# netapp-rickhuang-ai/spark-rapids-ml-nai

Hardware: AMD Instinct MI355X
Metric: fit-time speedup vs Spark-ML CPU (geomean over reference headline workloads, 1Mx3000 fp32) (higher is better)
Workload: dtype fp32

## Files before the change

spark_rapids_ml_nai_amd/ops/__init__.py:

```python
from __future__ import annotations

import math
import os
from typing import Any, Dict, Iterator, Optional, Tuple

import numpy as np
import torch

from . import native
from ..utils.determinism import deterministic

__all__ = ["col_moments", "gram", "xw", "dgemm", "sign_flip", "is_native", "xtv", "row_sqnorm",
           "logreg_binary_loss_grad", "nearest_centroid", "cluster_sums", "csr_logreg_binary_loss_grad",
           "csr_spmm", "csr_spmtm", "csr_col_moments", "logistic_loss_grad"]


def is_native(t: torch.Tensor) -> bool:
    return t.is_cuda


def _c(t: torch.Tensor) -> torch.Tensor:
    return t if t.is_contiguous() else t.contiguous()


# ... 419 lines not shown
    return labels, dist


_CERTIFY_STATS = {"rows": 0, "refined": 0}


F16_U = 2.0 ** -11
F16_A = 2.0 ** -14


def certify_tau16(n: int) -> float:
    return 1.01 * (2.0 * F16_U + F16_U * F16_U + 1.01 * float(n) * 2.0 ** -24)


def f16_radius_terms(n: int, scale: float, tau: float) -> Tuple[float, float, float]:
    a = F16_A / scale
    z = 2.02 * a * math.sqrt(n) * (1.0 + F16_U)
    z2 = 2.02 * float(n) * a * a
    wmax = math.sqrt(n) * 32768.0 / scale
    return (z + 2.0 ** -24 * wmax) / (2.0 * tau), z, z2


class F16Planes:

    def __init__(self, X: torch.Tensor, mu: torch.Tensor) -> None:
        m, n = X.shape
        self.X, self.m, self.n = X, m, n
        self.mu = _c(mu.float().view(-1))
        dev = X.device
        st = native.stream(dev)
        self.xnorm = torch.empty(m, dtype=torch.float32, device=dev)
        amax = zeros(1, dtype=torch.int32, device=dev)
        native.call("srml_row_sqnorm_centered_amax_f32", X.data_ptr(), m, n, X.stride(0), self.mu.data_ptr(),
                    self.xnorm.data_ptr(), amax.data_ptr(), st)
        a = float(amax.view(torch.float32).item())
        self.ok = math.isfinite(a) and a > 0.0
        self.scale = 1.0
        self.P = None
        if not self.ok:
            return
        e = math.frexp(a)[1] - 1
        if not -100 <= 13 - e <= 100:
            self.ok = False
            return
        self.scale = 2.0 ** (13 - e)
        self.kp = (n + 15) // 16 * 16
        self.rows_pad = max(256, (m + 255) // 256 * 256)
        self.P = torch.empty((self.rows_pad // 256, self.kp // 16, 256, 16), dtype=torch.float16, device=dev)
        self.ovf = zeros(1, dtype=torch.int32, device=dev)
        native.call("srml_split_f16_tiled_centered", X.data_ptr(), m, n, X.stride(0), self.mu.data_ptr(), self.kp,
                    self.rows_pad, self.scale, self.P.data_ptr(), self.ovf.data_ptr(), st)
        self.tau = certify_tau16(n)
        self.xadd, self.z, self.z2 = f16_radius_terms(n, self.scale, self.tau)


F16_CAND_CAP = 64


def _f16_centre_planes(F: F16Planes, C: torch.Tensor, approx: bool) -> Tuple[torch.Tensor, ...]:
    k, dev = C.shape[0], F.X.device
    st = native.stream(dev)
    Cd = _c(C.to(dev)) if C.dtype in (torch.float32, torch.float64) else _c(C.to(dev, torch.float32))
    crows = max(256, (k + 255) // 256 * 256)
    W = torch.empty((k, F.n), dtype=torch.float32, device=dev)
    cn = torch.empty(crows, dtype=torch.float32, device=dev)
    cg = torch.empty(k, dtype=torch.float32, device=dev)
    zero2 = torch.empty(2, dtype=torch.int32, device=dev)
    native.call("srml_f16_centre_prep", Cd.data_ptr(), int(Cd.dtype == torch.float64), k, F.n, F.mu.data_ptr(),
                float(2.0 * F.tau), int(bool(approx)), W.data_ptr(), cn.data_ptr(), cg.data_ptr(), zero2.data_ptr(), st)
    CP = torch.empty((crows // 256, F.kp // 16, 256, 16), dtype=torch.float16, device=dev)
    native.call("srml_split_f16_tiled_centered", W.data_ptr(), k, F.n, W.stride(0), None, F.kp, crows, F.scale,
                CP.data_ptr(), zero2[0:1].data_ptr(), st)
    return W, cn, cg, zero2, CP, crows


def nearest_f16_labels(F: F16Planes, C: torch.Tensor) -> Optional[torch.Tensor]:
    if F.kp != 128 or os.environ.get("SRML_F16_ROWLOOP", "1") == "0":
        return None
    dev = F.X.device
    _, cn, _, _, CP, crows = _f16_centre_planes(F, C, True)
    labels = torch.empty(F.m, dtype=torch.int32, device=dev)
    rc = native.lib().srml_nearest_f16_rowloop(F.P.data_ptr(), F.m, F.rows_pad, F.kp, CP.data_ptr(), C.shape[0],
                                                crows, cn.data_ptr(), float(-2.0 / (F.scale * F.scale)),
                                                labels.data_ptr(), native.stream(dev))
    if rc == -2:
        return None
    if rc != 0:
        raise RuntimeError("srml_nearest_f16_rowloop failed (%d)" % rc)
    return labels


def nearest_centroid_f16(F: F16Planes, C: torch.Tensor, approx: bool = False) -> Tuple[torch.Tensor, torch.Tensor]:
    m, k, dev = F.m, C.shape[0], F.X.device
    st = native.stream(dev)
    W, cn, cg, zero2, CP, crows = _f16_centre_planes(F, C, approx)
    ovf = zero2[0:1]
    xadd, z, z2 = (0.0, 0.0, 0.0) if approx else (F.xadd, F.z, F.z2)
    dscale = -2.0 / (F.scale * F.scale)
    nslot = int(native.lib().srml_nearest_centroid_f16_top2_nslot(k))
    labels = torch.empty(m, dtype=torch.int32, device=dev)
    dist = torch.empty(m, dtype=torch.float32, device=dev)
    flagged = torch.empty(m, dtype=torch.int32, device=dev)
    thr = torch.empty(m, dtype=torch.float32, device=dev)
    cnt = zero2[1:2]
    step = split_rows_per_launch(k)
    for r0 in range(0, m, step):
# ... 2147 lines not shown
```

spark_rapids_ml_nai_amd/ops/csrc/splitmm.hip:

```cpp
#include "common.h"

#include "tile.h"
#include <stdlib.h>

namespace {
using srml_tile::orderable;
using srml_tile::unorderable;

typedef short bf16x8 __attribute__((ext_vector_type(8)));
typedef _Float16 halfx8 __attribute__((ext_vector_type(8)));
typedef unsigned uintx4 __attribute__((ext_vector_type(4)));
typedef unsigned uintx2 __attribute__((ext_vector_type(2)));

__device__ __forceinline__ unsigned bf16_rn(float f) {
  unsigned u = __float_as_uint(f);
  u += 0x7fffu + ((u >> 16) & 1u);
  return u >> 16;
}
__device__ __forceinline__ float bf16_f(unsigned b) { return __uint_as_float(b << 16); }

__global__ __launch_bounds__(256) void split_kernel(const float* __restrict__ X, long m, int n, long ld, int kp,
                                                    long rows_pad, unsigned short* __restrict__ P) {
  const int q4 = kp >> 2;
  const long total = rows_pad * q4;
  const long plane = rows_pad * (long)kp;
  for (long i = (long)blockIdx.x * 256 + threadIdx.x; i < total; i += (long)gridDim.x * 256) {
    const long r = i / q4;
    const int c = (int)(i - r * q4) * 4;
    unsigned h[4], md[4], lo[4];
#pragma unroll
    for (int j = 0; j < 4; ++j) {
      const float x = (r < m && c + j < n) ? X[r * ld + c + j] : 0.f;
      h[j] = bf16_rn(x);
      const float r1 = x - bf16_f(h[j]);
      md[j] = bf16_rn(r1);
      lo[j] = bf16_rn(r1 - bf16_f(md[j]));
    }
    const long o = r * kp + c;
    *reinterpret_cast<uintx2*>(P + o) = uintx2{h[0] | (h[1] << 16), h[2] | (h[3] << 16)};
    *reinterpret_cast<uintx2*>(P + plane + o) = uintx2{md[0] | (md[1] << 16), md[2] | (md[3] << 16)};
    *reinterpret_cast<uintx2*>(P + 2 * plane + o) = uintx2{lo[0] | (lo[1] << 16), lo[2] | (lo[3] << 16)};
  }
}

__global__ __launch_bounds__(256) void split_tiled_kernel(const float* __restrict__ X, long m, int n, long ld, int kp,
                                                          long rows_pad, unsigned short* __restrict__ P,
                                                          const float* __restrict__ mu,
                                                          const int* __restrict__ ridx = nullptr) {
  const int ks_n = kp >> 4;
  const long total = rows_pad * ks_n;
  const long plane = rows_pad * (long)kp;
  const bool vec = (ld & 3) == 0 && (reinterpret_cast<uintptr_t>(X) & 15) == 0;
  for (long i = (long)blockIdx.x * 256 + threadIdx.x; i < total; i += (long)gridDim.x * 256) {
    const long img = i >> 8;
    const int rr = (int)(i & 255);
    const long tile = img / ks_n;
    const int c0 = (int)(img - tile * ks_n) * 16;
    const long r = tile * 256 + rr;
    const long rs = ridx && r < m ? (long)ridx[r] : r;
    float x[16];
    if (vec && r < m && c0 + 16 <= n) {
#pragma unroll
      for (int q = 0; q < 4; ++q) {
        const floatx4 v = *reinterpret_cast<const floatx4*>(X + rs * ld + c0 + 4 * q);
        x[4 * q] = v[0]; x[4 * q + 1] = v[1]; x[4 * q + 2] = v[2]; x[4 * q + 3] = v[3];
// ... 368 lines not shown
    for (int p = 0; p < 3; ++p) {
      a[p] = *reinterpret_cast<const uintx4*>(xa + p * xplane + ko);
      b[p] = *reinterpret_cast<const uintx4*>(ca + p * cplane + ko);
    }
  };
  auto lstore = [&](int stage, const uintx4 (&a)[3], const uintx4 (&b)[3]) {
#pragma unroll
    for (int p = 0; p < 3; ++p) {
      *reinterpret_cast<uintx4*>(&st[stage].A[p][sr][sh]) = a[p];
      *reinterpret_cast<uintx4*>(&st[stage].B[p][sr][sh]) = b[p];
    }
  };
  const int nk = kp / SBK;
  if (PF == 1) {
    uintx4 ra[3], rb[3];
    gload(0, ra, rb);
    lstore(0, ra, rb);
    __syncthreads();
    int cur = 0;
    for (int kt = 0; kt < nk; ++kt) {
      const bool more = kt + 1 < nk;
      if (more) gload(kt + 1, ra, rb);
      mma_step(cur);
      if (more) lstore(cur ^ 1, ra, rb);
      __syncthreads();
      cur ^= 1;
    }
  } else {
    uintx4 ra0[3], rb0[3], ra1[3], rb1[3];
    gload(0, ra0, rb0);
    if (nk > 1) gload(1, ra1, rb1);
    lstore(0, ra0, rb0);
    __syncthreads();
    int kt = 0;
    for (; kt + 2 <= nk; kt += 2) {
      if (kt + 2 < nk) gload(kt + 2, ra0, rb0);
      mma_step(0);
      lstore(1, ra1, rb1);
      __syncthreads();
      if (kt + 3 < nk) gload(kt + 3, ra1, rb1);
      mma_step(1);
      if (kt + 2 < nk) lstore(0, ra0, rb0);
      __syncthreads();
    }
    if (kt < nk) mma_step(0);
  }

  split_epilogue<BM, BN, WM, WN>(acc, row0, col0, m, k, cnorm, best, wm, wn, li, lk);
}

typedef __attribute__((address_space(3))) void* lds_vptr;
typedef __attribute__((address_space(1))) void* gbl_vptr;

template <bool TILED, int NP = 6, bool TOP2 = false, int WN_ = 4, bool PRIO = false, bool CAND = false, int RING = 0>
__global__ __launch_bounds__(WN_ * 128, WN_ == 4 ? 1 : 2) void nearest_centroid_split_glds_kernel(
    const unsigned short* __restrict__ XP, long m, long xrows, int kp, const unsigned short* __restrict__ CP, int k,
    long crows, const float* __restrict__ cnorm, unsigned long long* __restrict__ best, int n_ctiles,
    float* __restrict__ lob = nullptr, const float* __restrict__ cg = nullptr, const float* __restrict__ xnorm = nullptr,
    float dscale = -2.f, float xadd = 0.f, const float* __restrict__ thr = nullptr, int* __restrict__ ccount = nullptr,
    int* __restrict__ cand = nullptr, int cap = 0) {
  static_assert(!CAND || (NP == 1 && TOP2), "candidate lists come from the fp16 filter");
  static_assert(WN_ == 4 || (WN_ == 2 && NP != 6), "256 x 128 tiles are built for the filter passes");
  static_assert(NP == 6 || NP == 3 || (NP == 1 && TOP2), "NP = 1 is the fp16 certified filter");
  constexpr int BM = 256, WM = 2, WN = WN_, BN = 64 * WN, TM = 4, TN = 2;
  constexpr int NPL = NP == 6 ? 3 : (NP == 3 ? 2 : 1);
  constexpr int XCH = NPL * (BM / 32), CCH = NPL * (BN / 32);
  constexpr int CPW = (XCH + CCH) / (WM * WN);
  static_assert((XCH + CCH) % (WM * WN) == 0, "chunks split evenly over the waves");
  constexpr int KPB = RING ? RING / 10 : NP == 1 ? 3 : (NP == 3 && WN_ == 4 ? 2 : 1);
  constexpr int NG = RING ? RING % 10 : NP == 1 && WN_ == 4 ? 3 : 2;
  static_assert(!RING || (NP == 1 && KPB >= 1 && NG >= 2), "ring override is for the fp16 filter");
  constexpr int NS = (KPB > 1 || RING) ? NG * KPB : 3;
  constexpr int STAGE = NPL * (BM + BN) * 16;
  __shared__ __attribute__((aligned(1024))) unsigned short lds[NS][STAGE];
  const int bid = xcd_remap(blockIdx.x, gridDim.x);
  const long rtile = bid / n_ctiles;
  const int ctile = bid % n_ctiles;
  const long row0 = rtile * BM;
  const int col0 = ctile * BN;
  const int t = threadIdx.x;
  const int lane = t & 63, wid = t >> 6;
  const int wm = wid / WN, wn = wid % WN;
  const int li = lane & 31, lk = lane >> 5;
  const long xplane = xrows * (long)kp, cplane = crows * (long)kp;

  const unsigned short* src[CPW];
  int dst_off[CPW];
#pragma unroll
  for (int i = 0; i < CPW; ++i) {
    const int c = wid * CPW + i;
    const bool isx = c < XCH;
    const int q = isx ? c / (BM / 32) : (c - XCH) / (BN / 32);
    const int j = isx ? c % (BM / 32) : (c - XCH) % (BN / 32);
    const int r = 32 * j + (lane >> 1);
    const int lh = (lane & 1) ^ ((lane >> 4) & 1);
    if (TILED) {
      const int ks_n = kp / SBK;
      if (isx) src[i] = XP + q * xplane + ((rtile * ks_n) << 12) + 512 * j + lane * 8;
      else src[i] = CP + q * cplane + (((long)(col0 >> 8) * ks_n) << 12) + 16 * (col0 & 255) + 512 * j + lane * 8;
    } else if (isx) {
      long xr = row0 + r;
      if (xr >= xrows) xr = xrows - 1;
      src[i] = XP + q * xplane + xr * kp + 8 * lh;
    } else {
      src[i] = CP + q * cplane + (long)(col0 + r) * kp + 8 * lh;
    }
    dst_off[i] = isx ? (q * BM + 32 * j) * 16 : (NPL * BM + q * BN + 32 * j) * 16;
  }
  auto issue = [&](int kt, int stage) {
    unsigned short* base = &lds[stage][0];
#pragma unroll
    for (int i = 0; i < CPW; ++i) {
      __builtin_amdgcn_global_load_lds((gbl_vptr)(src[i] + (TILED ? ((long)kt << 12) : (long)kt * SBK)),
                                       (lds_vptr)(base + dst_off[i]), 16, 0, 0);
    }
  };

  floatx16 acc[TM][TN];
#pragma unroll
  for (int a = 0; a < TM; ++a)
#pragma unroll
    for (int b = 0; b < TN; ++b)
#pragma unroll
      for (int r = 0; r < 16; ++r) acc[a][b][r] = 0.f;

  const int ph = lk ^ ((li >> 3) & 1);
  const int nk = kp / SBK;
  auto compute = [&](int st) {
    bf16x8 fb[NPL][TN];
#pragma unroll
    for (int p = 0; p < NPL; ++p)
#pragma unroll
      for (int nt = 0; nt < TN; ++nt)
        fb[p][nt] = *reinterpret_cast<const bf16x8*>(
            &lds[st][(NPL * BM + p * BN + wn * (BN / WN) + nt * 32 + li) * 16 + 8 * ph]);
#pragma unroll
    for (int mt = 0; mt < TM; ++mt) {
      bf16x8 fa[NPL];
#pragma unroll
      for (int p = 0; p < NPL; ++p)
        fa[p] = *reinterpret_cast<const bf16x8*>(&lds[st][(p * BM + wm * (BM / WM) + mt * 32 + li) * 16 + 8 * ph]);
#pragma unroll
      for (int nt = 0; nt < TN; ++nt) {
        if constexpr (NP == 1) {
          acc[mt][nt] = __builtin_amdgcn_mfma_f32_32x32x16_f16(__builtin_bit_cast(halfx8, fb[0][nt]),
                                                               __builtin_bit_cast(halfx8, fa[0]), acc[mt][nt], 0,
                                                               0, 0);
        } else {
          if constexpr (NP == 6) {
            acc[mt][nt] = __builtin_amdgcn_mfma_f32_32x32x16_bf16(fa[2], fb[0][nt], acc[mt][nt], 0, 0, 0);
            acc[mt][nt] = __builtin_amdgcn_mfma_f32_32x32x16_bf16(fa[1], fb[1][nt], acc[mt][nt], 0, 0, 0);
            acc[mt][nt] = __builtin_amdgcn_mfma_f32_32x32x16_bf16(fa[0], fb[2][nt], acc[mt][nt], 0, 0, 0);
          }
          acc[mt][nt] = __builtin_amdgcn_mfma_f32_32x32x16_bf16(fa[1], fb[0][nt], acc[mt][nt], 0, 0, 0);
          acc[mt][nt] = __builtin_amdgcn_mfma_f32_32x32x16_bf16(fa[0], fb[1][nt], acc[mt][nt], 0, 0, 0);
          acc[mt][nt] = __builtin_amdgcn_mfma_f32_32x32x16_bf16(fa[0], fb[0][nt], acc[mt][nt], 0, 0, 0);
        }
      }
    }
  };
  if constexpr (KPB == 1 && !RING) {
    static_assert(CPW == 6, "the counted wait below leaves one step (CPW loads) in flight");
    issue(0, 0);
    if (nk > 1) issue(1, 1);
    int stage = 0;
    for (int kt = 0; kt < nk; ++kt) {
      if (kt + 1 < nk) asm volatile("s_waitcnt vmcnt(6)" ::: "memory");
      else asm volatile("s_waitcnt vmcnt(0)" ::: "memory");
      __builtin_amdgcn_s_barrier();
      if (kt + 2 < nk) issue(kt + 2, stage == 0 ? 2 : stage - 1);
      if (PRIO) __builtin_amdgcn_s_setprio(1);
      compute(stage);
      if (PRIO) __builtin_amdgcn_s_setprio(0);
      stage = stage == 2 ? 0 : stage + 1;
    }
  } else {
#pragma unroll
    for (int j = 0; j < (NG - 1) * KPB; ++j)
      if (j < nk) issue(j, j);
    for (int kt = 0; kt < nk; kt += KPB) {
      if (NG >= 3 && kt + (NG - 1) * KPB <= nk)
        asm volatile("s_waitcnt vmcnt(%0)" ::"i"((NG - 2) * KPB * CPW) : "memory");
      else asm volatile("s_waitcnt vmcnt(0)" ::: "memory");
      __builtin_amdgcn_s_barrier();
#pragma unroll
      for (int j = 0; j < KPB; ++j)
        if (kt + (NG - 1) * KPB + j < nk) issue(kt + (NG - 1) * KPB + j, (kt + (NG - 1) * KPB + j) % NS);
      if (PRIO) __builtin_amdgcn_s_setprio(1);
#pragma unroll
      for (int j = 0; j < KPB; ++j)
        if (kt + j < nk) compute((kt + j) % NS);
      if (PRIO) __builtin_amdgcn_s_setprio(0);
    }
  }
  if (CAND)
    split_epilogue_cand_t<BM, BN, WM, WN>(acc, row0, col0, m, k, cnorm, cg, xnorm, wm, wn, li, lk, dscale, xadd, thr,
                                          ccount, cand, cap);
  else if (TOP2 && NP == 1)
    split_epilogue_top2_t<BM, BN, WM, WN>(acc, row0, col0, ctile, m, k, cnorm, cg, xnorm, best, lob, n_ctiles * WN, wm,
                                          wn, li, lk, dscale, xadd);
  else if (TOP2)
    split_epilogue_top2<BM, BN, WM, WN>(acc, row0, col0, ctile, m, k, cnorm, cg, xnorm, best, lob, n_ctiles * WN, wm,
                                        wn, li, lk, dscale, xadd);
  else
    split_epilogue<BM, BN, WM, WN>(acc, row0, col0, m, k, cnorm, best, wm, wn, li, lk);
}

__global__ __launch_bounds__(256) void split_top2_select_kernel(const unsigned long long* __restrict__ keys,
                                                                const float* __restrict__ lob, long m, int nslot,
                                                                const float* __restrict__ xnorm,
                                                                const float* __restrict__ cg,
                                                                int* __restrict__ labels, float* __restrict__ dist,
                                                                int* __restrict__ flagged, int* __restrict__ n_flagged,
                                                                float xadd = 0.f, float z = 0.f, float z2 = 0.f,
                                                                const int* __restrict__ ovf = nullptr,
                                                                float* __restrict__ thr_out = nullptr) {
  const long i = (long)blockIdx.x * 256 + threadIdx.x;
  if (i >= m) return;
  unsigned long long k1 = ~0ull;
  int s1 = 0;
  for (int s = 0; s < nslot; ++s) {
    const unsigned long long v = keys[(long)s * m + i];
    if (v < k1) { k1 = v; s1 = s; }
  }
  const float xn = xnorm[i];
  const float xs0 = sqrtf(fmaxf(xn, 0.f));
  const float xs = xs0 + xadd;
  const float c2 = 2.f * fmaf(z, xs0, z2);
  float low = __builtin_huge_valf();
  for (int s = 0; s < nslot; ++s) {
    low = fminf(low, lob[(long)s * m + i]);
    const unsigned long long v = keys[(long)s * m + i];
    if (s != s1 && v != ~0ull) low = fminf(low, fmaf(-xs, cg[(int)(v & 0xffffffffu)], unorderable((unsigned)(v >> 32))));
  }
  const float bv = unorderable((unsigned)(k1 >> 32));
  if (k1 != ~0ull && !(ovf && *ovf) && low > fmaf(xs, cg[(int)(k1 & 0xffffffffu)], bv) + c2) {
    labels[i] = (int)(k1 & 0xffffffffu);
    const float d = bv + xn;
    dist[i] = d > 0.f ? d : 0.f;
  } else {
    const int p = atomicAdd(n_flagged, 1);
    flagged[p] = (int)i;
    if (thr_out)
      thr_out[p] = (k1 != ~0ull && !(ovf && *ovf)) ? fmaf(xs, cg[(int)(k1 & 0xffffffffu)], bv) + c2
                                                   : __builtin_huge_valf();
  }
}
// ... 220 lines not shown
  return srml_nearest_centroid_split_tiled_np(XP, m, xrows, kp, CP, k, crows, cnorm, best, 6, stream);
}

SRML_API int srml_nearest_centroid_split_top2(const unsigned short* XP, long m, long xrows, int kp,
                                              const unsigned short* CP, int k, long crows, const float* cnorm,
                                              const float* cg, const float* xnorm, unsigned long long* keys,
                                              float* lob, hipStream_t stream) {
  if (m <= 0 || k <= 0) return 0;
  if ((kp & 15) || xrows < m || crows < k || (crows & 255) || (xrows & 255)) return -2;
  if ((reinterpret_cast<uintptr_t>(XP) & 15) || (reinterpret_cast<uintptr_t>(CP) & 15)) return -5;
  const long rt = (m + 255) / 256;
  const int bn = split3_bn();
  const int ct = (k + bn - 1) / bn;
  const long nb = rt * ct;
  if (nb > srml_max_blocks(512)) return -3;
  static const bool prio = !(getenv("SRML_SPLIT_PRIO") && atoi(getenv("SRML_SPLIT_PRIO")) == 0);
#define SRML_TOP2(WNN, PR, T)                                                                                    \
  hipLaunchKernelGGL((nearest_centroid_split_glds_kernel<true, 3, true, WNN, PR>), dim3((unsigned)nb), dim3(T), 0, \
                     stream, XP, m, xrows, kp, CP, k, crows, cnorm, keys, (int)ct, lob, cg, xnorm)
  if (bn == 128 && prio) SRML_TOP2(2, true, 256);
  else if (bn == 128) SRML_TOP2(2, false, 256);
  else if (prio) SRML_TOP2(4, true, 512);
  else SRML_TOP2(4, false, 512);
#undef SRML_TOP2
  return srml_status();
}

SRML_API int srml_nearest_centroid_split_top2_nslot(int k) {
  const int bn = split3_bn();
  return ((k + bn - 1) / bn) * (bn / 64);
}

SRML_API int srml_split_top2_select(const unsigned long long* keys, const float* lob, long m, int nslot,
                                    const float* xnorm, const float* cg, int* labels, float* dist, int* flagged,
                                    int* n_flagged, hipStream_t stream) {
  if (m <= 0) return 0;
  hipLaunchKernelGGL(split_top2_select_kernel, dim3((unsigned)((m + 255) / 256)), dim3(256), 0, stream, keys, lob, m,
                     nslot, xnorm, cg, labels, dist, flagged, n_flagged);
  return srml_status();
}

SRML_API int srml_split_scatter_refined(const unsigned long long* best, const int* rows, int nf, const float* xnorm,
                                        int* labels, float* dist, hipStream_t stream) {
  if (nf <= 0) return 0;
  hipLaunchKernelGGL(split_scatter_refined_kernel, dim3((unsigned)((nf + 255) / 256)), dim3(256), 0, stream, best,
                     rows, nf, xnorm, labels, dist);
  return srml_status();
}

static int f16_bn() {
  static const int bn = getenv("SRML_F16_BN") && atoi(getenv("SRML_F16_BN")) == 128 ? 128 : 256;
  return bn;
}
static int f16_slots_per_tile() { return f16_bn() / 64; }

template <typename T>
__global__ __launch_bounds__(256) void f16_centre_prep_kernel(const T* __restrict__ C, int k, int n,
                                                              const float* __restrict__ mu, float tau2, int approx,
                                                              float* __restrict__ W, float* __restrict__ cn,
                                                              float* __restrict__ cg, int* __restrict__ zero2) {
  const int j = blockIdx.x * 4 + (threadIdx.x >> 6);
  const int lane = threadIdx.x & 63;
  if (blockIdx.x == 0 && threadIdx.x < 2) zero2[threadIdx.x] = 0;
  if (j >= k) return;
  double a = 0.0;
  for (int d = lane; d < n; d += 64) {
    const float w = (float)((double)C[(long)j * n + d] - (double)mu[d]);
    W[(long)j * n + d] = w;
    a += (double)w * (double)w;
  }
  for (int o = 32; o > 0; o >>= 1) a += __shfl_xor(a, o, 64);
  if (lane == 0) {
    const float c = (float)a;
    cn[j] = c;
    cg[j] = approx ? 0.f : tau2 * sqrtf(c > 0.f ? c : 0.f);
  }
}

SRML_API int srml_f16_centre_prep(const void* C, int c_f64, int k, int n, const float* mu, float tau2, int approx,
                                  float* W, float* cn, float* cg, int* zero2, hipStream_t stream) {
  if (k <= 0) return 0;
  const dim3 grid((unsigned)((k + 3) / 4));
  if (c_f64)
    hipLaunchKernelGGL(f16_centre_prep_kernel<double>, grid, dim3(256), 0, stream,
                       reinterpret_cast<const double*>(C), k, n, mu, tau2, approx, W, cn, cg, zero2);
  else
    hipLaunchKernelGGL(f16_centre_prep_kernel<float>, grid, dim3(256), 0, stream, reinterpret_cast<const float*>(C),
                       k, n, mu, tau2, approx, W, cn, cg, zero2);
  return srml_status();
}

SRML_API int srml_split_f16_tiled_centered(const float* X, long m, int n, long ld, const float* mu, int kp,
                                           long rows_pad, float scale, unsigned short* P, int* ovf,
                                           hipStream_t stream) {
  if (rows_pad <= 0) return 0;
  if ((kp & 15) || kp < n || rows_pad < m || (rows_pad & 255)) return -2;
  if ((reinterpret_cast<uintptr_t>(P) & 15) != 0) return -5;
  const long total = rows_pad * (long)(kp / 16);
  long blocks = (total + 255) / 256;
  if (blocks > 65536) blocks = 65536;
  hipLaunchKernelGGL(split_tiled_f16_kernel, dim3((unsigned)blocks), dim3(256), 0, stream, X, m, n, ld, kp, rows_pad, P,
                     mu, scale, ovf);
  return srml_status();
}

SRML_API int srml_nearest_centroid_f16_top2(const unsigned short* XP, long m, long xrows, int kp,
                                            const unsigned short* CP, int k, long crows, const float* cnorm,
                                            const float* cg, const float* xnorm, float dscale, float xadd,
                                            unsigned long long* keys, float* lob, hipStream_t stream) {
  if (m <= 0 || k <= 0) return 0;
  if ((kp & 15) || xrows < m || crows < k || (crows & 255) || (xrows & 255)) return -2;
  if ((reinterpret_cast<uintptr_t>(XP) & 15) || (reinterpret_cast<uintptr_t>(CP) & 15)) return -5;
  const long rt = (m + 255) / 256;
  const int bn = f16_bn();
  const int ct = (k + bn - 1) / bn;
  const long nb = rt * ct;
  if (nb > srml_max_blocks(bn * 2)) return -3;
  static const bool prio = !(getenv("SRML_SPLIT_PRIO") && atoi(getenv("SRML_SPLIT_PRIO")) == 0);
#define SRML_F16(WNN, PR, T)                                                                                      \
  hipLaunchKernelGGL((nearest_centroid_split_glds_kernel<true, 1, true, WNN, PR>), dim3((unsigned)nb), dim3(T), 0, \
                     stream, XP, m, xrows, kp, CP, k, crows, cnorm, keys, (int)ct, lob, cg, xnorm, dscale, xadd)
  static const int ring = getenv("SRML_F16_RING") ? atoi(getenv("SRML_F16_RING")) : 0;
#define SRML_F16R(RG)                                                                                               \
  hipLaunchKernelGGL((nearest_centroid_split_glds_kernel<true, 1, true, 4, true, false, RG>), dim3((unsigned)nb),      \
                     dim3(512), 0, stream, XP, m, xrows, kp, CP, k, crows, cnorm, keys, (int)ct, lob, cg, xnorm,       \
                     dscale, xadd)
  if (f16_bn() == 128) {
    if (prio) SRML_F16(2, true, 256);
    else SRML_F16(2, false, 256);
  } else if (ring == 23) {
    SRML_F16R(23);
  } else if (ring == 24) {
    SRML_F16R(24);
  } else if (ring == 42) {
    SRML_F16R(42);
  } else if (ring == 18) {
    SRML_F16R(18);
  } else if (ring == 25) {
    SRML_F16R(25);
  } else {
    if (prio) SRML_F16(4, true, 512);
    else SRML_F16(4, false, 512);
  }
#undef SRML_F16R
#undef SRML_F16
  return srml_status();
}

SRML_API int srml_nearest_centroid_f16_top2_nslot(int k) {
  const int bn = f16_bn();
  return ((k + bn - 1) / bn) * f16_slots_per_tile();
}

SRML_API int srml_split_top2_select_f16(const unsigned long long* keys, const float* lob, long m, int nslot,
                                        const float* xnorm, const float* cg, float xadd, float z, float z2,
                                        const int* ovf, int* labels, float* dist, int* flagged, int* n_flagged,
                                        hipStream_t stream) {
  if (m <= 0) return 0;
  hipLaunchKernelGGL(split_top2_select_kernel, dim3((unsigned)((m + 255) / 256)), dim3(256), 0, stream, keys, lob, m,
                     nslot, xnorm, cg, labels, dist, flagged, n_flagged, xadd, z, z2, ovf);
  return srml_status();
}

SRML_API int srml_split_f16_tiled_centered_rows(const float* X, long ld, const int* ridx, long m, int n,
                                                const float* mu, int kp, long rows_pad, float scale, unsigned short* P,
                                                int* ovf, hipStream_t stream) {
  if (rows_pad <= 0) return 0;
  if ((kp & 15) || kp < n || rows_pad < m || (rows_pad & 255) || !ridx) return -2;
  if ((reinterpret_cast<uintptr_t>(P) & 15) != 0) return -5;
  const long total = rows_pad * (long)(kp / 16);
  long blocks = (total + 255) / 256;
  if (blocks > 65536) blocks = 65536;
  hipLaunchKernelGGL(split_tiled_f16_kernel, dim3((unsigned)blocks), dim3(256), 0, stream, X, m, n, ld, kp, rows_pad, P,
                     mu, scale, ovf, ridx);
  return srml_status();
}

__global__ __launch_bounds__(256) void f16_plane_gather_kernel(const uintx4* __restrict__ src, int ks_n,
                                                               const int* __restrict__ ridx, long m, long rows_pad,
                                                               uintx4* __restrict__ dst,
                                                               const float* __restrict__ xn = nullptr,
                                                               float* __restrict__ xn_out = nullptr,
                                                               int* __restrict__ zero_out = nullptr) {
  for (long i = (long)blockIdx.x * 256 + threadIdx.x; i < m; i += (long)gridDim.x * 256) {
    if (xn_out) xn_out[i] = xn[ridx[i]];
    if (zero_out) zero_out[i] = 0;
  }
  const long total = rows_pad * ks_n;
  for (long i = (long)blockIdx.x * 256 + threadIdx.x; i < total; i += (long)gridDim.x * 256) {
    const long img = i >> 8;
    const int rr = (int)(i & 255);
    const long tile = img / ks_n;
    const long ks = img - tile * ks_n;
    const long r = tile * 256 + rr;
    uintx4 lo = uintx4{0u, 0u, 0u, 0u}, hi = lo;
    if (r < m) {
// ... 2 lines not shown
      const uintx4* s = src + ((((rs >> 8) * ks_n + ks) << 12) + (rs & 255) * 16) / 8;
      lo = s[ssw];
      hi = s[ssw ^ 1];
    }
    const int dsw = (rr >> 3) & 1;
    uintx4* d = dst + ((img << 12) + rr * 16) / 8;
    d[dsw] = lo;
    d[dsw ^ 1] = hi;
  }
}

SRML_API int srml_f16_plane_gather_rows_ex(const unsigned short* P, long src_rows_pad, int kp, const int* ridx, long m,
                                           long rows_pad, unsigned short* out, const float* xn, float* xn_out,
                                           int* zero_out, hipStream_t stream) {
  if (rows_pad <= 0) return 0;
  if ((kp & 15) || rows_pad < m || (rows_pad & 255) || (src_rows_pad & 255) || !ridx) return -2;
  if ((reinterpret_cast<uintptr_t>(P) & 15) || (reinterpret_cast<uintptr_t>(out) & 15)) return -5;
  if (xn_out && !xn) return -2;
  const long total = rows_pad * (long)(kp / 16);
  long blocks = (total + 255) / 256;
  if (blocks > 65536) blocks = 65536;
  hipLaunchKernelGGL(f16_plane_gather_kernel, dim3((unsigned)blocks), dim3(256), 0, stream,
                     reinterpret_cast<const uintx4*>(P), kp / 16, ridx, m, rows_pad, reinterpret_cast<uintx4*>(out), xn,
                     xn_out, zero_out);
  return srml_status();
}

SRML_API int srml_f16_plane_gather_rows(const unsigned short* P, long src_rows_pad, int kp, const int* ridx, long m,
                                        long rows_pad, unsigned short* out, hipStream_t stream) {
  return srml_f16_plane_gather_rows_ex(P, src_rows_pad, kp, ridx, m, rows_pad, out, nullptr, nullptr, nullptr, stream);
}

SRML_API int srml_split_top2_select_f16_thr(const unsigned long long* keys, const float* lob, long m, int nslot,
                                            const float* xnorm, const float* cg, float xadd, float z, float z2,
                                            const int* ovf, int* labels, float* dist, int* flagged, int* n_flagged,
                                            float* thr_out, hipStream_t stream) {
  if (m <= 0) return 0;
  hipLaunchKernelGGL(split_top2_select_kernel, dim3((unsigned)((m + 255) / 256)), dim3(256), 0, stream, keys, lob, m,
                     nslot, xnorm, cg, labels, dist, flagged, n_flagged, xadd, z, z2, ovf, thr_out);
  return srml_status();
}

SRML_API int srml_nearest_centroid_f16_cand(const unsigned short* XP, long m, long xrows, int kp,
                                            const unsigned short* CP, int k, long crows, const float* cnorm,
                                            const float* cg, const float* xnorm, float dscale, float xadd,
                                            const float* thr, int* ccount, int* cand, int cap, hipStream_t stream) {
  if (m <= 0 || k <= 0) return 0;
  if ((kp & 15) || xrows < m || crows < k || (crows & 255) || (xrows & 255) || cap < 1) return -2;
  if ((reinterpret_cast<uintptr_t>(XP) & 15) || (reinterpret_cast<uintptr_t>(CP) & 15)) return -5;
  const long rt = (m + 255) / 256;
  const int ct = (k + 255) / 256;
  const long nb = rt * ct;
  if (nb > srml_max_blocks(512)) return -3;
  hipLaunchKernelGGL((nearest_centroid_split_glds_kernel<true, 1, true, 4, true, true>), dim3((unsigned)nb), dim3(512),
                     0, stream, XP, m, xrows, kp, CP, k, crows, cnorm, (unsigned long long*)nullptr, (int)ct,
                     (float*)nullptr, cg, xnorm, dscale, xadd, thr, ccount, cand, cap);
  return srml_status();
}

SRML_API int srml_kmeans_cand_exact(const float* X, long ld, const float* mu, const float* W, long ldw, int n, int k,
                                    const int* rows, int nf, const int* ccount, const int* cand, int cap, int* labels,
                                    float* dist, hipStream_t stream) {
  if (nf <= 0) return 0;
  const dim3 grid((unsigned)((nf + 3) / 4));
  const bool vec = (n & 3) == 0 && (ld & 3) == 0 && (ldw & 3) == 0 && (reinterpret_cast<uintptr_t>(X) & 15) == 0 &&
                   (reinterpret_cast<uintptr_t>(W) & 15) == 0 && (reinterpret_cast<uintptr_t>(mu) & 15) == 0;
  const int nv = (n / 4 + 63) / 64;
  static const bool scalar = getenv("SRML_CAND_EXACT") && atoi(getenv("SRML_CAND_EXACT")) == 0;
#define SRML_CE(NVV)                                                                                                  \
  hipLaunchKernelGGL(cand_exact_vec_kernel<NVV>, grid, dim3(256), 0, stream, X, ld, mu, W, ldw, n, k, rows, nf, ccount, \
                     cand, cap, labels, dist)
  if (vec && !scalar && nv <= 4) SRML_CE(4);
  else if (vec && !scalar && nv <= 8) SRML_CE(8);
  else if (vec && !scalar && nv <= 12) SRML_CE(12);
  else if (vec && !scalar && nv <= 16) SRML_CE(16);
  else
    hipLaunchKernelGGL(cand_exact_kernel, grid, dim3(256), 0, stream, X, ld, mu, W, ldw, n, k, rows, nf, ccount, cand,
                       cap, labels, dist);
#undef SRML_CE
  return srml_status();
}

namespace {
template <int KS>
__global__ __launch_bounds__(512, 1) void nearest_f16_rowloop_kernel(const unsigned short* __restrict__ XP, long m,
                                                                     const unsigned short* __restrict__ CP, int k,
                                                                     int n_ctiles, const float* __restrict__ cnorm,
                                                                     float dscale, int* __restrict__ labels) {
  constexpr int CT = 256;
  constexpr int IMG = CT * 16;
  constexpr int CHUNKS = KS * 8;
  constexpr int CPW = CHUNKS / 8;
  __shared__ __attribute__((aligned(1024))) unsigned short lds[2][KS * IMG];
  __shared__ __attribute__((aligned(1024))) float cn_s[2][CT];
  const long tile = xcd_remap(blockIdx.x, gridDim.x);
  const int t = threadIdx.x, lane = t & 63, wid = t >> 6, li = lane & 31, lk = lane >> 5;
  const int rr = 32 * wid + li;
  halfx8 xb[KS];
#pragma unroll
  for (int ks = 0; ks < KS; ++ks)
    xb[ks] = *reinterpret_cast<const halfx8*>(XP + ((tile * KS + ks) << 12) + rr * 16 + 8 * (lk ^ ((rr >> 3) & 1)));
  auto issue = [&](int c, int buf) {
    const unsigned short* src = CP + ((long)c * KS << 12);
#pragma unroll
    for (int i = 0; i < CPW; ++i) {
      const int ch = wid * CPW + i;
      __builtin_amdgcn_global_load_lds((gbl_vptr)(src + ch * 512 + lane * 8), (lds_vptr)(&lds[buf][ch * 512]), 16, 0,
                                       0);
    }
// ... 78 lines not shown
```

spark_rapids_ml_nai_amd/ops/native.py:

```python
from __future__ import annotations

import ctypes
import os
import threading
from typing import Any, Dict, Optional, Tuple

import torch

from . import build as _build

_P = ctypes.c_void_p
_I = ctypes.c_int
_L = ctypes.c_long
_D = ctypes.c_double
_F = ctypes.c_float

_LONG_RESULT = ("srml_rf_bootstrap_ws", "srml_logreg_fold_ws", "srml_qn_mb_scratch", "srml_qn_fused_scratch",
                "srml_qn_fused_barrier_offset",
                "srml_logreg_fold_parts", "srml_qn_args_size", "srml_logit_residual_ws", "srml_xtv_mfma_ws",
                "srml_rf_partition_ws", "srml_dbscan_labels_ws", "srml_umap_categorical_ws",
                "srml_label_sort_ws", "srml_radix_sort_ws", "srml_lloyd_moved_ws", "srml_sum_f32_ws", "srml_sum_sq_ws")
SIGNATURES: Dict[str, Tuple[Any, ...]] = {
    "srml_col_moments_f32": (_P, _L, _I, _L, _P, _P, _P),
    "srml_col_moments_f64": (_P, _L, _I, _L, _P, _P, _P),
# ... 15 lines not shown
    "srml_logreg_fold_ws": (_L, _I, _L, _P),
    "srml_logreg_zcache_ok": (_L, _I, _L, _P),
    "srml_logreg_binary_lds_f32": (_P, _L, _I, _L, _P, _P, _D, _P, _P, _P, _P),
    "srml_logreg_binary_lds_f64": (_P, _L, _I, _L, _P, _P, _D, _P, _P, _P, _P),
    "srml_xtv2_f32": (_P, _L, _I, _L, _P, _I, _L, _P, _L, _L, _P, _P),
    "srml_xtv_mfma_f32": (_P, _L, _I, _L, _P, _I, _L, _P, _L, _L, _P, _P),
    "srml_xtv_mfma_det_f32": (_P, _L, _I, _L, _P, _I, _L, _P, _L, _L, _P, _P, _P),
    "srml_fold_partials_f64": (_P, _L, _L, _L, _L, _P, _L, _L, _P, _P),
    "srml_xw_t_f32": (_P, _L, _I, _L, _P, _I, _L, _P, _P, _L, _P),
    "srml_xw_t_f32_skip": (_P, _L, _I, _L, _P, _I, _L, _P, _P, _L, _P, _P),
    "srml_xw_t_f32_variant": (_P, _L, _I, _L, _P, _I, _L, _P, _P, _L, _I, _P),
    "srml_logit_residual_f32": (_P, _L, _I, _L, _P, _P, _L, _I, _P, _L, _P, _L, _P, _L, _P, _P),
    "srml_logit_residual_zc_f32": (_P, _L, _I, _L, _P, _P, _L, _I, _P, _L, _P, _L, _P, _L, _P, _P, _P, _P, _P),
    "srml_logit_residual_f64": (_P, _L, _I, _L, _P, _P, _L, _I, _P, _L, _P, _L, _P, _L, _P, _P),
    "srml_logit_residual_det_f32": (_P, _L, _I, _L, _P, _P, _L, _I, _P, _L, _P, _L, _P, _L, _P, _P, _P),
    "srml_logit_residual_ws": (_L, _I),
    "srml_xtv_mfma_ws": (_L, _I, _I),
    "srml_mbin_f32": (_P, _L, _I, _L, _P, _P, _L, _I, _P, _L, _P),
    "srml_qn_step_batch": (_P, _I, _P),
    "srml_mlogit_f32": (_P, _L, _I, _L, _P, _P, _P, _P, _I, _P, _P),
    "srml_mlogit_supported": (_I, _I),
    "srml_qn_step": (_P, _P),
    "srml_qn_step_mb": (_P, _P, _P),
    "srml_qn_step_fused": (_P, _P, _P, _I, _L, _P),
    "srml_qn_step_mbf": (_P, _P, _P, _I, _L, _P),
    "srml_kmeans_lloyd_small": (_P, _L, _I, _L, _P, _I, _P, _P, _P, _P, _P, _P, _P),
    "srml_kmeans_lloyd_mfma": (_P, _L, _I, _L, _P, _I, _P, _P, _P, _P, _P, _P, _P, _P, _P),
    "srml_kmeans_small_update": (_P, _I, _I, _P, _P, _P, _D, _P, _P, _P, _P),
    "srml_qn_fused_scratch": (),
    "srml_qn_fused_barrier_offset": (),
    "srml_qn_fused_resident": (_L,),
    "srml_qn_mb_scratch": (),
    "srml_kmeanspp_gram": (_P, _I, _L, _P, _I, _I, ctypes.c_ulonglong, _P, _P),
    "srml_qn_max_history": (),
    "srml_qn_args_size": (),
    "srml_nearest_centroid_f32": (_P, _L, _I, _L, _P, _I, _L, _P, _P, _P),
    "srml_nn_finalize": (_P, _L, _P, _P, _P, _P),
    "srml_split_bf16x3": (_P, _L, _I, _L, _I, _L, _P, _P),
    "srml_nearest_centroid_split": (_P, _L, _L, _I, _P, _I, _L, _P, _P, _P),
    "srml_split_bf16x3_tiled": (_P, _L, _I, _L, _I, _L, _P, _P),
    "srml_nearest_centroid_split_tiled": (_P, _L, _L, _I, _P, _I, _L, _P, _P, _P),
    "srml_nearest_centroid_split_tiled_np": (_P, _L, _L, _I, _P, _I, _L, _P, _P, _I, _P),
    "srml_nearest_centroid_split_top2": (_P, _L, _L, _I, _P, _I, _L, _P, _P, _P, _P, _P, _P),
    "srml_split_bf16x3_tiled_centered": (_P, _L, _I, _L, _P, _I, _L, _P, _P),
    "srml_split_bf16x3_tiled_centered_rows": (_P, _L, _P, _L, _I, _P, _I, _L, _P, _P),
    "srml_row_sqnorm_centered_f32": (_P, _L, _I, _L, _P, _P, _P),
    "srml_row_sqnorm_centered_amax_f32": (_P, _L, _I, _L, _P, _P, _P, _P),
    "srml_rf_sample_features_floyd": (_I, _I),
    "srml_rf_bootstrap_ws": (_I, _L),
    "srml_rf_bootstrap": (_I, _L, _D, ctypes.c_ulonglong, _P, _P, _P, _P, _P),
    "srml_split_f16_tiled_centered": (_P, _L, _I, _L, _P, _I, _L, _F, _P, _P, _P),
    "srml_nearest_centroid_f16_top2": (_P, _L, _L, _I, _P, _I, _L, _P, _P, _P, _F, _F, _P, _P, _P),
    "srml_nearest_centroid_f16_top2_nslot": (_I,),
    "srml_split_top2_select_f16": (_P, _P, _L, _I, _P, _P, _F, _F, _F, _P, _P, _P, _P, _P, _P),
    "srml_split_f16_tiled_centered_rows": (_P, _L, _P, _L, _I, _P, _I, _L, _F, _P, _P, _P),
    "srml_f16_plane_gather_rows": (_P, _L, _I, _P, _L, _L, _P, _P),
    "srml_nearest_f16_rowloop": (_P, _L, _L, _I, _P, _I, _L, _P, _F, _P, _P),
    "srml_f16_plane_gather_rows_ex": (_P, _L, _I, _P, _L, _L, _P, _P, _P, _P, _P),
    "srml_split_top2_select_f16_thr": (_P, _P, _L, _I, _P, _P, _F, _F, _F, _P, _P, _P, _P, _P, _P, _P),
    "srml_nearest_centroid_f16_cand": (_P, _L, _L, _I, _P, _I, _L, _P, _P, _P, _F, _F, _P, _P, _P, _I, _P),
    "srml_kmeans_cand_exact": (_P, _L, _P, _P, _L, _I, _I, _P, _I, _P, _P, _I, _P, _P, _P),
    "srml_nearest_centroid_split_top2_nslot": (_I,),
    "srml_split_top2_select": (_P, _P, _L, _I, _P, _P, _P, _P, _P, _P, _P),
    "srml_split_scatter_refined": (_P, _P, _I, _P, _P, _P, _P),
    "srml_kmeans_accumulate_f32": (_P, _L, _I, _L, _P, _I, _P, _P, _P, _P),
    "srml_kmeans_accumulate_sorted_f32": (_P, _L, _I, _L, _P, _P, _P, _P),
    "srml_kmeans_accumulate_sorted_rows_f32": (_P, _L, _I, _L, _P, _P, _P, _P, _P),
    "srml_lloyd_moved_ws": (_L,),
    "srml_lloyd_moved_count": (_P, _P, _L, _P, _P, _P),
    "srml_lloyd_moved_compact": (_P, _P, _L, _P, _L, _P, _P, _P, _P),
    "srml_counts_from_offsets": (_P, _I, _P, _P),
    "srml_sum_f32_ws": (),
    "srml_sum_f32_f64": (_P, _L, _P, _P, _P),
    "srml_lloyd_centre_update": (_P, _I, _I, _P, _P, _P, _P),
    "srml_kmeans_segment_sums_f32": (_P, _L, _I, _L, _P, _P, _I, _P, _I, _P, _P),
    "srml_kmeans_segment_sums_f64": (_P, _L, _I, _L, _P, _P, _I, _P, _I, _P, _P),
    "srml_nearest_centroid_f64": (_P, _L, _I, _L, _P, _I, _L, _P, _P, _P, _P, _P, _P),
    "srml_row_sqnorm_f64": (_P, _L, _I, _L, _P, _P),
    "srml_knn_dist_f32": (_P, _L, _I, _L, _P, _L, _L, _P, _P, _L, _P),
    "srml_topk_rows_f32": (_P, _L, _L, _L, _I, _P, _L, ctypes.c_longlong, _I, _P, _P, _L, _L, _P),
    "srml_knn_f32": (_P, _L, _I, _L, _P, _L, _L, _P, _I, _I, _P, _P, ctypes.c_longlong, _P),
    "srml_ivf_search_f32": (_P, _L, _I, _L, _P, _I, _P, _P, _L, _P, _P, _I, _P, _P, _P),
    "srml_knn_lists_f32": (_P, _I, _L, _P, _P, _P, _I, _P, _P, _I, _I, _P, _P, _P),
    "srml_f16_centre_prep": (_P, _I, _I, _I, _P, _F, _I, _P, _P, _P, _P, _P),
    "srml_knn_lists_f16c": (_P, _I, _L, _P, _P, _P, _I, _P, _P, _I, _I, _P, _P, _P),
    "srml_knn_pairs_f16c": (_P, _I, _L, _P, _P, _P, _P, _P, _P, _P, _I, _I, _P, _P, _P, _P, _P, _P, _P),
    "srml_center_rows_f16": (_P, _I, _L, _P, _P, _I, _L, _P, _P, _P),
    "srml_dbscan_degree_f32": (_P, _L, _I, _L, _P, _F, _L, _L, _P, _P),
    "srml_dbscan_link_f32": (_P, _L, _I, _L, _P, _F, _L, _L, _P, _P, _P, _P),
    "srml_uf_unite_pairs": (_P, _L, _P, _P),
    "srml_uf_compress": (_P, _L, _P),
    "srml_dbscan_labels_ws": (_L,),
    "srml_umap_categorical_ws": (_L, _L),
    "srml_umap_categorical": (_P, _P, _P, _L, _P, _L, _D, _D, _D, _P, _P, _P),
    "srml_dbscan_labels": (_P, _P, _P, _L, _P, _P, _P),
    "srml_oneshot_alloc": (_L, _P, _P),
    "srml_oneshot_open": (_P, _P),
    "srml_oneshot_close": (_P,),
    "srml_oneshot_free": (_P,),
    "srml_oneshot_allreduce": (_P, _P, _L, _I, _P, _I, _I, ctypes.c_ulonglong, _L, ctypes.c_longlong, _P, _P),
    "srml_umap_smooth_knn": (_P, _P, _L, _I, _L, _D, _D, _I, _P, _I, _P, _P, _P, _P),
    "srml_umap_fuzzy_union_knn": (_P, _P, _L, _I, _L, ctypes.c_float, _P, _P, _P, _P),
    "srml_umap_epoch": (_P, _P, _L, _P, _P, _P, _P, _P, _P, _I, _I, _F, _F, _F, _F, _F, _I, _I, ctypes.c_uint, _P, _P,
                        _I, _P),
    "srml_umap_neg_table": (_P, _P, _L, _I, _P, _P),
    "srml_syevj_f64": (_P, _I, _P, _P, _I, _D, _P),
# ... 135 lines not shown
```

Before: 3498.

## Add software-pipelined fp16 filter main loop with register fragment prefetch

Adds a SCHED=1 variant of the fp16 nearest-centroid filter kernel (256x256 tile, ring 2x4). It double-buffers LDS fragments in registers, reading the next step's fragments and issuing the global-to-LDS DMA between individual MFMAs under sched barriers, with one barrier per group. The variant is on by default for both the top2 and candidate paths and can be switched off with an env var or a Python setter. The aim is to hide LDS read and DMA issue latency behind MFMA work, at the cost of extra registers and more complex wait-count logic. Optional timestamp instrumentation is compiled in only under a macro.

```diff
diff --git a/spark_rapids_ml_nai_amd/ops/__init__.py b/spark_rapids_ml_nai_amd/ops/__init__.py
--- a/spark_rapids_ml_nai_amd/ops/__init__.py
+++ b/spark_rapids_ml_nai_amd/ops/__init__.py
@@ -495,6 +495,15 @@
                     self.rows_pad, self.scale, self.P.data_ptr(), self.ovf.data_ptr(), st)
         self.tau = certify_tau16(n)
         self.xadd, self.z, self.z2 = f16_radius_terms(n, self.scale, self.tau)
+
+
+F16_SCHEDULES = (0, 1)
+
+
+def f16_sched(sched: Optional[int] = None) -> int:
+    if sched is not None and sched not in F16_SCHEDULES:
+        raise ValueError("f16_sched: unknown schedule %r" % (sched,))
+    return int(native.lib().srml_f16_sched(-1 if sched is None else int(sched)))
 
 
 F16_CAND_CAP = 64
diff --git a/spark_rapids_ml_nai_amd/ops/csrc/splitmm.hip b/spark_rapids_ml_nai_amd/ops/csrc/splitmm.hip
--- a/spark_rapids_ml_nai_amd/ops/csrc/splitmm.hip
+++ b/spark_rapids_ml_nai_amd/ops/csrc/splitmm.hip
@@ -11,6 +11,20 @@
 typedef _Float16 halfx8 __attribute__((ext_vector_type(8)));
 typedef unsigned uintx4 __attribute__((ext_vector_type(4)));
 typedef unsigned uintx2 __attribute__((ext_vector_type(2)));
+
+#ifdef SRML_F16_STAMPS
+__device__ unsigned long long f16_stamp_sums[8];
+#define F16_STAMP(t)                                                                 \
+  do {                                                                               \
+    __builtin_amdgcn_sched_barrier(0);                                               \
+    asm volatile("s_memtime %0\n\ts_waitcnt lgkmcnt(0)" : "=s"(t)::"memory");       \
+    __builtin_amdgcn_sched_barrier(0);                                               \
+  } while (0)
+#define F16_STAMP_ADD(i, d) (tsum[i] += (d))
+#else
+#define F16_STAMP(t) ((void)0)
+#define F16_STAMP_ADD(i, d) ((void)0)
+#endif
 
 __device__ __forceinline__ unsigned bf16_rn(float f) {
   unsigned u = __float_as_uint(f);
@@ -485,7 +499,8 @@
 typedef __attribute__((address_space(3))) void* lds_vptr;
 typedef __attribute__((address_space(1))) void* gbl_vptr;
 
-template <bool TILED, int NP = 6, bool TOP2 = false, int WN_ = 4, bool PRIO = false, bool CAND = false, int RING = 0>
+template <bool TILED, int NP = 6, bool TOP2 = false, int WN_ = 4, bool PRIO = false, bool CAND = false, int RING = 0,
+          int SCHED = 0>
 __global__ __launch_bounds__(WN_ * 128, WN_ == 4 ? 1 : 2) void nearest_centroid_split_glds_kernel(
     const unsigned short* __restrict__ XP, long m, long xrows, int kp, const unsigned short* __restrict__ CP, int k,
     long crows, const float* __restrict__ cnorm, unsigned long long* __restrict__ best, int n_ctiles,
@@ -495,6 +510,7 @@
   static_assert(!CAND || (NP == 1 && TOP2), "candidate lists come from the fp16 filter");
   static_assert(WN_ == 4 || (WN_ == 2 && NP != 6), "256 x 128 tiles are built for the filter passes");
   static_assert(NP == 6 || NP == 3 || (NP == 1 && TOP2), "NP = 1 is the fp16 certified filter");
+  static_assert(!SCHED || (NP == 1 && WN_ == 4 && TILED && RING), "the prefetching loop is the 256 x 256 fp16 filter's");
   constexpr int BM = 256, WM = 2, WN = WN_, BN = 64 * WN, TM = 4, TN = 2;
   constexpr int NPL = NP == 6 ? 3 : (NP == 3 ? 2 : 1);
   constexpr int XCH = NPL * (BM / 32), CCH = NPL * (BN / 32);
@@ -503,6 +519,7 @@
   constexpr int KPB = RING ? RING / 10 : NP == 1 ? 3 : (NP == 3 && WN_ == 4 ? 2 : 1);
   constexpr int NG = RING ? RING % 10 : NP == 1 && WN_ == 4 ? 3 : 2;
   static_assert(!RING || (NP == 1 && KPB >= 1 && NG >= 2), "ring override is for the fp16 filter");
+  static_assert(!SCHED || (NG >= 4 && KPB % 2 == 0), "prefetching loop: >= 4 groups of an even number of k steps");
   constexpr int NS = (KPB > 1 || RING) ? NG * KPB : 3;
   constexpr int STAGE = NPL * (BM + BN) * 16;
   __shared__ __attribute__((aligned(1024))) unsigned short lds[NS][STAGE];
@@ -557,6 +574,9 @@
 #pragma unroll
       for (int r = 0; r < 16; ++r) acc[a][b][r] = 0.f;
 
+#ifdef SRML_F16_STAMPS
+  unsigned long long ts[5] = {0, 0, 0, 0, 0}, tsum[5] = {0, 0, 0, 0, 0};
+#endif
   const int ph = lk ^ ((li >> 3) & 1);
   const int nk = kp / SBK;
   auto compute = [&](int st) {
@@ -592,7 +612,99 @@
       }
     }
   };
-  if constexpr (KPB == 1 && !RING) {
+  if constexpr (SCHED == 1) {
+    constexpr int NF = TM + TN;
+    bf16x8 F[2][NF];
+    auto frag_read1 = [&](bf16x8 (&f)[NF], int st, int i) {
+      const int r = i < TN ? BM + wn * (BN / WN) + i * 32 + li : wm * (BM / WM) + (i - TN) * 32 + li;
+      f[i] = *reinterpret_cast<const bf16x8*>(&lds[st][r * 16 + 8 * ph]);
+    };
+    auto step = [&](const bf16x8 (&f)[NF], bf16x8 (&fn)[NF], int st, auto rd, auto is, int kti, int sti) {
+      constexpr bool READ = decltype(rd)::value;
+      constexpr bool ISSUE = decltype(is)::value;
+      __builtin_amdgcn_sched_barrier(0);
+      asm volatile("s_waitcnt lgkmcnt(0)" ::: "memory");
+      __builtin_amdgcn_sched_barrier(0);
+      __builtin_amdgcn_s_setprio(1);
+#pragma unroll
+      for (int mt = 0; mt < TM; ++mt)
+#pragma unroll
+        for (int nt = 0; nt < TN; ++nt) {
+          acc[mt][nt] = __builtin_amdgcn_mfma_f32_32x32x16_f16(__builtin_bit_cast(halfx8, f[nt]),
+                                                               __builtin_bit_cast(halfx8, f[TN + mt]), acc[mt][nt],
+                                                               0, 0, 0);
+          if (READ && mt * TN + nt < NF) {
+            __builtin_amdgcn_sched_barrier(0);
+            frag_read1(fn, st, mt * TN + nt);
+            __builtin_amdgcn_sched_barrier(0);
+          }
+          if (ISSUE && mt * TN + nt >= NF && mt * TN + nt - NF < KPB) {
+            __builtin_amdgcn_sched_barrier(0);
+            issue(kti + mt * TN + nt - NF, sti + mt * TN + nt - NF);
+            __builtin_amdgcn_sched_barrier(0);
+          }
+        }
+      __builtin_amdgcn_s_setprio(0);
+      __builtin_amdgcn_sched_barrier(0);
+    };
+    static_assert(NF <= TM * TN, "one read behind each of the first NF MFMAs");
+#pragma unroll
+    for (int j = 0; j < (NG - 1) * KPB; ++j)
+      if (j < nk) issue(j, j);
+    if ((NG - 1) * KPB <= nk) asm volatile("s_waitcnt vmcnt(%0)" ::"i"((NG - 2) * KPB * CPW) : "memory");
+    else asm volatile("s_waitcnt vmcnt(0)" ::: "memory");
+    __builtin_amdgcn_s_barrier();
+    asm volatile("" ::: "memory");
+#pragma unroll
+    for (int i = 0; i < NF; ++i) frag_read1(F[0], 0, i);
+    const int ngf = nk / KPB;
+    int st0 = 0;
+    int g = 0;
+    static_assert(NF + KPB <= TM * TN, "one DMA step behind each MFMA after the reads");
+    for (; (g + NG) * KPB <= nk; ++g) {
+      F16_STAMP(ts[0]);
+      asm volatile("s_waitcnt vmcnt(%0)" ::"i"((NG - 3) * KPB * CPW) : "memory");
+      F16_STAMP(ts[1]);
+      __builtin_amdgcn_s_barrier();
+      asm volatile("" ::: "memory");
+      F16_STAMP(ts[2]);
+      const int stn = st0 + KPB == NS ? 0 : st0 + KPB;
+      const int str = st0 == 0 ? NS - KPB : st0 - KPB;
+      step(F[0], F[1], st0 + 1, std::true_type{}, std::true_type{}, (g + NG - 1) * KPB, str);
+#pragma unroll
+      for (int j = 1; j < KPB; ++j)
+        step(F[j & 1], F[(j + 1) & 1], j + 1 < KPB ? st0 + j + 1 : stn, std::true_type{}, std::false_type{}, 0, 0);
+      st0 = stn;
+      F16_STAMP(ts[3]);
+      F16_STAMP_ADD(0, ts[1] - ts[0]);
+      F16_STAMP_ADD(1, ts[2] - ts[1]);
+      F16_STAMP_ADD(3, ts[3] - ts[2]);
+      F16_STAMP_ADD(4, 1);
+    }
+    for (; g < ngf; ++g) {
+      const int kt = g * KPB;
+      if (kt + (NG - 1) * KPB <= nk) asm volatile("s_waitcnt vmcnt(%0)" ::"i"((NG - 3) * KPB * CPW) : "memory");
+      else asm volatile("s_waitcnt vmcnt(0)" ::: "memory");
+      __builtin_amdgcn_s_barrier();
+      asm volatile("" ::: "memory");
+      const int stn = st0 + KPB == NS ? 0 : st0 + KPB;
+      const int str = st0 == 0 ? NS - KPB : st0 - KPB;
+#pragma unroll
+      for (int j = 0; j < KPB; ++j)
+        if (kt + (NG - 1) * KPB + j < nk) issue(kt + (NG - 1) * KPB + j, str + j);
+#pragma unroll
+      for (int j = 0; j < KPB; ++j)
+        step(F[j & 1], F[(j + 1) & 1], j + 1 < KPB ? st0 + j + 1 : stn, std::true_type{}, std::false_type{}, 0, 0);
+      st0 = stn;
+    }
+    for (int j = 0; j < nk - ngf * KPB; ++j) {
+      if (j) {
+#pragma unroll
+        for (int i = 0; i < NF; ++i) frag_read1(F[0], st0 + j, i);
+      }
+      step(F[0], F[1], 0, std::false_type{}, std::false_type{}, 0, 0);
+    }
+  } else if constexpr (KPB == 1 && !RING) {
     static_assert(CPW == 6, "the counted wait below leaves one step (CPW loads) in flight");
     issue(0, 0);
     if (nk > 1) issue(1, 1);
@@ -612,20 +724,37 @@
     for (int j = 0; j < (NG - 1) * KPB; ++j)
       if (j < nk) issue(j, j);
     for (int kt = 0; kt < nk; kt += KPB) {
+      F16_STAMP(ts[0]);
       if (NG >= 3 && kt + (NG - 1) * KPB <= nk)
         asm volatile("s_waitcnt vmcnt(%0)" ::"i"((NG - 2) * KPB * CPW) : "memory");
       else asm volatile("s_waitcnt vmcnt(0)" ::: "memory");
+      F16_STAMP(ts[1]);
       __builtin_amdgcn_s_barrier();
+      F16_STAMP(ts[2]);
 #pragma unroll
       for (int j = 0; j < KPB; ++j)
         if (kt + (NG - 1) * KPB + j < nk) issue(kt + (NG - 1) * KPB + j, (kt + (NG - 1) * KPB + j) % NS);
+      F16_STAMP(ts[3]);
       if (PRIO) __builtin_amdgcn_s_setprio(1);
 #pragma unroll
       for (int j = 0; j < KPB; ++j)
         if (kt + j < nk) compute((kt + j) % NS);
       if (PRIO) __builtin_amdgcn_s_setprio(0);
-    }
-  }
+      F16_STAMP(ts[4]);
+      F16_STAMP_ADD(0, ts[1] - ts[0]);
+      F16_STAMP_ADD(1, ts[2] - ts[1]);
+      F16_STAMP_ADD(2, ts[3] - ts[2]);
+      F16_STAMP_ADD(3, ts[4] - ts[3]);
+      F16_STAMP_ADD(4, 1);
+    }
+  }
+#ifdef SRML_F16_STAMPS
+  if (NP == 1 && t == 0) {
+#pragma unroll
+    for (int i = 0; i < 5; ++i) atomicAdd(&f16_stamp_sums[i], tsum[i]);
+    atomicAdd(&f16_stamp_sums[5], 1ull);
+  }
+#endif
   if (CAND)
     split_epilogue_cand_t<BM, BN, WM, WN>(acc, row0, col0, m, k, cnorm, cg, xnorm, wm, wn, li, lk, dscale, xadd, thr,
                                           ccount, cand, cap);
@@ -952,6 +1081,26 @@
   static const int bn = getenv("SRML_F16_BN") && atoi(getenv("SRML_F16_BN")) == 128 ? 128 : 256;
   return bn;
 }
+constexpr int F16_SCHED_DEFAULT = 1;
+static int& f16_sched_ref() {
+  static int s = (getenv("SRML_F16_SCHED") ? atoi(getenv("SRML_F16_SCHED")) : F16_SCHED_DEFAULT) == 1 ? 1 : 0;
+  return s;
+}
+static int f16_sched() { return f16_sched_ref(); }
+SRML_API int srml_f16_sched(int sched) {
+  if (sched == 0 || sched == 1) f16_sched_ref() = sched;
+  return f16_sched();
+}
+#ifdef SRML_F16_STAMPS
+SRML_API int srml_f16_stamps(unsigned long long* out, int reset) {
+  if (hipMemcpyFromSymbol(out, HIP_SYMBOL(f16_stamp_sums), sizeof(f16_stamp_sums)) != hipSuccess) return -1;
+  if (reset) {
+    const unsigned long long z[8] = {0, 0, 0, 0, 0, 0, 0, 0};
+    if (hipMemcpyToSymbol(HIP_SYMBOL(f16_stamp_sums), z, sizeof(z)) != hipSuccess) return -1;
+  }
+  return 0;
+}
+#endif
 static int f16_slots_per_tile() { return f16_bn() / 64; }
 
 template <typename T>
@@ -1025,9 +1174,15 @@
   hipLaunchKernelGGL((nearest_centroid_split_glds_kernel<true, 1, true, 4, true, false, RG>), dim3((unsigned)nb),      \
                      dim3(512), 0, stream, XP, m, xrows, kp, CP, k, crows, cnorm, keys, (int)ct, lob, cg, xnorm,       \
                      dscale, xadd)
+#define SRML_F16S()                                                                                                 \
+  hipLaunchKernelGGL((nearest_centroid_split_glds_kernel<true, 1, true, 4, true, false, 24, 1>), dim3((unsigned)nb),   \
+                     dim3(512), 0, stream, XP, m, xrows, kp, CP, k, crows, cnorm, keys, (int)ct, lob, cg, xnorm,       \
+                     dscale, xadd)
   if (f16_bn() == 128) {
     if (prio) SRML_F16(2, true, 256);
     else SRML_F16(2, false, 256);
+  } else if (f16_sched() == 1) {
+    SRML_F16S();
   } else if (ring == 23) {
     SRML_F16R(23);
   } else if (ring == 24) {
@@ -1042,6 +1197,7 @@
     if (prio) SRML_F16(4, true, 512);
     else SRML_F16(4, false, 512);
   }
+#undef SRML_F16S
 #undef SRML_F16R
 #undef SRML_F16
   return srml_status();
@@ -1150,9 +1306,14 @@
   const int ct = (k + 255) / 256;
   const long nb = rt * ct;
   if (nb > srml_max_blocks(512)) return -3;
-  hipLaunchKernelGGL((nearest_centroid_split_glds_kernel<true, 1, true, 4, true, true>), dim3((unsigned)nb), dim3(512),
-                     0, stream, XP, m, xrows, kp, CP, k, crows, cnorm, (unsigned long long*)nullptr, (int)ct,
-                     (float*)nullptr, cg, xnorm, dscale, xadd, thr, ccount, cand, cap);
+  if (f16_sched() == 1)
+    hipLaunchKernelGGL((nearest_centroid_split_glds_kernel<true, 1, true, 4, true, true, 24, 1>), dim3((unsigned)nb),
+                       dim3(512), 0, stream, XP, m, xrows, kp, CP, k, crows, cnorm, (unsigned long long*)nullptr,
+                       (int)ct, (float*)nullptr, cg, xnorm, dscale, xadd, thr, ccount, cand, cap);
+  else
+    hipLaunchKernelGGL((nearest_centroid_split_glds_kernel<true, 1, true, 4, true, true>), dim3((unsigned)nb),
+                       dim3(512), 0, stream, XP, m, xrows, kp, CP, k, crows, cnorm, (unsigned long long*)nullptr,
+                       (int)ct, (float*)nullptr, cg, xnorm, dscale, xadd, thr, ccount, cand, cap);
   return srml_status();
 }
 
diff --git a/spark_rapids_ml_nai_amd/ops/native.py b/spark_rapids_ml_nai_amd/ops/native.py
--- a/spark_rapids_ml_nai_amd/ops/native.py
+++ b/spark_rapids_ml_nai_amd/ops/native.py
@@ -91,6 +91,7 @@
     "srml_split_f16_tiled_centered": (_P, _L, _I, _L, _P, _I, _L, _F, _P, _P, _P),
     "srml_nearest_centroid_f16_top2": (_P, _L, _L, _I, _P, _I, _L, _P, _P, _P, _F, _F, _P, _P, _P),
     "srml_nearest_centroid_f16_top2_nslot": (_I,),
+    "srml_f16_sched": (_I,),
     "srml_split_top2_select_f16": (_P, _P, _L, _I, _P, _P, _F, _F, _F, _P, _P, _P, _P, _P, _P),
     "srml_split_f16_tiled_centered_rows": (_P, _L, _P, _L, _I, _P, _I, _L, _F, _P, _P, _P),
     "srml_f16_plane_gather_rows": (_P, _L, _I, _P, _L, _L, _P, _P),
```

After: 3527 (median of 6 runs). No clear change (+0.8%).
